# HiKapok/DAN

Measured on NVIDIA B200. Metric: images/sec anchor match+encode+decode+NMS @640^2, higher is better.
Workload: dtype f32

## Files before the change

### dan_b200/csrc/postprocess.cu

```cuda
#include <math.h>
#include <stdlib.h>
#include <string.h>

#include "common.cuh"

namespace dan {

#ifdef DAN_PHASE_TIMING
__device__ long long g_phase[32];
#define DAN_PHASE(slot) do { if (threadIdx.x == 0 && blockIdx.x == 0 && blockIdx.y == 0) g_phase[slot] = clock64(); } while (0)
#else
#define DAN_PHASE(slot) do { } while (0)
#endif

#ifndef DAN_PP_THREADS
#define DAN_PP_THREADS 1024
#endif
#define DAN_SORT_THREADS DAN_PP_THREADS
#include "sort.cuh"

struct PpArgs {
  const float* cls;
  const float4* loc;
  const float4* boxes;
  const float* ay0;
  const float* ax0;
  const float* ay1;
  const float* ax1;
  int n, batch, num_classes;
  float img_h, img_w;
  float select_thr, min_size_p1;
  float reject_below;
  float ps0, ps1, ps2, ps3;
  int keep_topk, nms_topk;
  int nms_cap;
  float nms_thr;
  int sort_bytes, kcap, wcap, cand_global, kept_global;
  int kstride;
  int dyn_smem_bytes;
  unsigned long long* keys;
  int32_t* key_count;
  int32_t* maybe;
  float4* stash;
  float* s_scores;
  float4* s_boxes;
  int32_t* s_index;
  unsigned long long* s_key;
  unsigned long long* s_key2;
  float4* s_box;
  float* s_area;
  float4* g_kept_box;
// ... 199 lines not shown
  r.area = fmul(fsub(r.y1, r.y0), fsub(r.x1, r.x0));
  return r;
}

__device__ __noinline__ bool nms_suppresses(float4 a, float a_area, float4 b, float b_area, float thr) {
  if (a_area <= 0.f || b_area <= 0.f) return false;
  const float h = fmaxf(fsub(fminf(a.z, b.z), fmaxf(a.x, b.x)), 0.f);
  const float w = fmaxf(fsub(fminf(a.w, b.w), fmaxf(a.y, b.y)), 0.f);
  const float inter = fmul(h, w);
  if (inter == 0.f) return 0.f > thr;
  return fdiv(inter, fsub(fadd(a_area, b_area), inter)) > thr;
}

DAN_D bool pair_suppresses(const float4& a, float a_area, const float4& b, float b_area, float thr) {
  if (thr >= 0.f) {
    const float h = fsub(fminf(a.z, b.z), fmaxf(a.x, b.x));
    const float w = fsub(fminf(a.w, b.w), fmaxf(a.y, b.y));
    if (!(h > 0.f && w > 0.f)) return false;
    if (!(a_area > 0.f && b_area > 0.f)) return false;
    const float inter = fmul(h, w);
    const float t = fmul(thr, fsub(fadd(a_area, b_area), inter));
    if (t > 1e-30f) {
      if (inter > fmul(t, 1.000001f)) return true;
      if (inter < fmul(t, 0.999999f)) return false;
    }
  }
  return nms_suppresses(a, a_area, b, b_area, thr);
}

DAN_D bool f2_maybe(const PpArgs& A, float x0, float x1) {
  return !(fsub(x1, x0) < A.reject_below) || fabsf(x0) > 1e5f || fabsf(x1) > 1e5f;
}

constexpr int kWin = kSortThreads;
#ifndef DAN_NMS_SURV
#define DAN_NMS_SURV 128
#endif
constexpr int kSurv = DAN_NMS_SURV;
constexpr int kSurvWords = kSurv / 32;
constexpr int kMaxSweeps = 12;
constexpr int kHintCells = 32 * 32;
constexpr size_t kGreedySmemMax = 186 * 1024;

struct GreedyPlan {
  size_t smem;
  int sort_bytes;
  int kcap;
  int wcap;
  int cand_global;
  int kept_global;
};

static int next_pow2(int64_t v) {
  int p = 1;
  while (p < v) p <<= 1;
  return p;
}

static GreedyPlan greedy_plan(int64_t n, int keep_topk, int nms_cap) {
  GreedyPlan g;
  const int sort_n = (int)(n < kSortCap ? (n > 0 ? n : 1) : kSortCap);
  g.sort_bytes = next_pow2(sort_n) * 8;
  g.kcap = (int)(keep_topk < n ? keep_topk : (n > 0 ? n : 1));
  g.wcap = (nms_cap + 31) / 32;
  const size_t kept_bytes = align_up((size_t)nms_cap * 16, 16) + 2 * align_up((size_t)nms_cap * 4, 16) + (size_t)64 * g.wcap * 4;
  const size_t cand_box = align_up((size_t)g.kcap * 16, 16);
  const size_t region0 = cand_box > (size_t)g.sort_bytes ? cand_box : (size_t)g.sort_bytes;
  const size_t full = region0 + align_up((size_t)g.kcap * 4, 16) + align_up((size_t)g.kcap * 8, 16) + kept_bytes;
  g.cand_global = g.kept_global = 0;
  g.smem = full;
  if (full > kGreedySmemMax) {
    g.cand_global = 1;
    g.smem = (size_t)g.sort_bytes + kept_bytes;
    if (g.smem > kGreedySmemMax) {
      g.kept_global = 1;
      g.smem = (size_t)g.sort_bytes;
    }
  }
  return g;
}

DAN_D void block_minmax(float lo, float hi, float& out_lo, float& out_hi) {
  __shared__ int s_lo[kSortThreads / 32], s_hi[kSortThreads / 32];
  const int lane = threadIdx.x & 31, warp = threadIdx.x >> 5;
  const int wl = __reduce_min_sync(0xffffffffu, float_to_ordered(lo));
  const int wh = __reduce_max_sync(0xffffffffu, float_to_ordered(hi));
  if (lane == 0) { s_lo[warp] = wl; s_hi[warp] = wh; }
  __syncthreads();
  int a = (lane < kSortThreads / 32) ? s_lo[lane] : 0x7fffffff, b = (lane < kSortThreads / 32) ? s_hi[lane] : (int)0x80000000;
  a = __reduce_min_sync(0xffffffffu, a);
  b = __reduce_max_sync(0xffffffffu, b);
  out_lo = ordered_to_float(a);
  out_hi = ordered_to_float(b);
  __syncthreads();
}

struct Stripes {
  float ylo, yinv, xlo, xinv;
  bool all;
  DAN_D static uint32_t axis(float v0, float v1, float lo, float inv) {
    const float f0 = (v0 - lo) * inv, f1 = (v1 - lo) * inv;
    if (!(fabsf(f0) < 1e9f) || !(fabsf(f1) < 1e9f)) return 0xffffffffu;
    const int s0 = min(max((int)f0, 0), 31), s1 = min(max((int)f1, 0), 31);
    return (0xffffffffu >> (31 - s1)) & (0xffffffffu << s0);
  }
  DAN_D uint2 masks(float4 bx, float area) const {
    if (!(area > 0.f)) return make_uint2(0u, 0u);
    if (all) return make_uint2(0xffffffffu, 0xffffffffu);
    return make_uint2(axis(bx.y, bx.w, xlo, xinv), axis(bx.x, bx.z, ylo, yinv));
  }
  DAN_D int cell(float4 bx) const {
    const float fy = ((bx.x + bx.z) * 0.5f - ylo) * yinv, fx = ((bx.y + bx.w) * 0.5f - xlo) * xinv;
    const int sy = (fabsf(fy) < 1e9f) ? min(max((int)fy, 0), 31) : 0;
    const int sx = (fabsf(fx) < 1e9f) ? min(max((int)fx, 0), 31) : 0;
    return sy * 32 + sx;
  }
};

DAN_D void bar_sync_chunk() { asm volatile("bar.sync 1, %0;" ::"n"(kSurv) : "memory"); }
DAN_D bool bar_or_chunk(bool pred) {
  int r;
  asm volatile(
      "{\n"
      "  .reg .pred p, q;\n"
      "  setp.ne.s32 q, %1, 0;\n"
      "  bar.red.or.pred p, 1, %2, q;\n"
      "  selp.s32 %0, 1, 0, p;\n"
      "}\n"
      : "=r"(r)
      : "r"((int)pred), "n"(kSurv)
      : "memory");
  return r != 0;
}

__device__ __noinline__ void resolve_chunk_serially(const uint32_t* T, uint32_t* keptm, uint32_t* supm, int ns) {
  const int lane = threadIdx.x & 31;
  uint32_t kw = (lane < kSurvWords) ? keptm[lane] : 0u;
  uint32_t sw = (lane < kSurvWords) ? supm[lane] : 0u;
  for (int v = 0; v < ns; ++v) {
    const int w = v >> 5;
    const uint32_t bit = 1u << (v & 31);
    const uint32_t known = __shfl_sync(0xffffffffu, kw | sw, w);
    if (known & bit) continue;
    const uint32_t t = (lane < kSurvWords && (lane << 5) < v) ? T[v * kSurvWords + lane] : 0u;
    const bool hit = __any_sync(0xffffffffu, (t & kw) != 0u);
    if (lane == w) {
      if (hit) sw |= bit;
      else kw |= bit;
    }
  }
  if (lane < kSurvWords) { keptm[lane] = kw; supm[lane] = sw; }
}

#ifndef DAN_NMS_REGS
#define DAN_NMS_BOUNDS __launch_bounds__(kSortThreads, 1024 / kSortThreads)
#else
#define DAN_NMS_BOUNDS __maxnreg__(DAN_NMS_REGS)
#endif
constexpr int kMaybeCap = 4096;

template <bool DECODE, int WHERE, bool FILTER>
__global__ void DAN_NMS_BOUNDS nms_greedy_kernel(const PpArgs A, const float* __restrict__ src_scores,
                                                                     const float4* __restrict__ src_boxes) {
  extern __shared__ __align__(16) unsigned char dyn_smem[];
  __shared__ SortScratch sc;
  __shared__ unsigned char s_alive[kWin];
  __shared__ unsigned short s_list[kWin];
  __shared__ int s_surv[kSurv];
  __shared__ float4 s_sbox[kSurv];
  __shared__ float s_sarea[kSurv];
  __shared__ uint32_t s_T[kSurv][kSurvWords];
  __shared__ uint32_t s_keptm[kSurvWords], s_supm[kSurvWords];
  __shared__ uint2 s_smask[kSurv];
  __shared__ int s_hint[2][kHintCells];
  __shared__ int s_wcnt[kSortThreads / 32];
  __shared__ int s_next[2];
  __shared__ int s_nlist, s_cnext;

  const int list = blockIdx.x;
  const int tid = threadIdx.x;
  const int lane = tid & 31;
  const int warp = tid >> 5;
  const unsigned lt_mask = (1u << lane) - 1u;
  const int b = list / max(A.num_classes - 1, 1);
  const int64_t o = (int64_t)list * A.kstride;
  const float thr = A.nms_thr;

  unsigned long long* keys = reinterpret_cast<unsigned long long*>(dyn_smem);
  float4* cbox;
  float* carea;
  uint2* cmask;
  unsigned char* p;
  if (WHERE >= 1) {
    cbox = A.s_box + o;
    carea = A.s_area + o;
    cmask = A.s_mask + o;
    p = dyn_smem + A.sort_bytes;
  } else {
    const size_t cand_box = ((size_t)A.kcap * 16 + 15) / 16 * 16;
    cbox = reinterpret_cast<float4*>(dyn_smem);
    carea = reinterpret_cast<float*>(dyn_smem + (cand_box > (size_t)A.sort_bytes ? cand_box : (size_t)A.sort_bytes));
    cmask = reinterpret_cast<uint2*>(reinterpret_cast<unsigned char*>(carea) + ((size_t)A.kcap * 4 + 15) / 16 * 16);
    p = reinterpret_cast<unsigned char*>(cmask) + ((size_t)A.kcap * 8 + 15) / 16 * 16;
  }
  float4* kbox;
  float* karea;
  int* krank;
  uint32_t* stripes;
// ... 2 lines not shown
    const int64_t ok = (int64_t)list * A.kstride;
    kbox = A.g_kept_box + ok;
    karea = A.g_kept_area + ok;
    krank = A.g_kept_rank + ok;
    stripes = A.g_stripes + (int64_t)list * 64 * ((A.kstride + 31) / 32);
  } else {
    kbox = reinterpret_cast<float4*>(p); p += ((size_t)A.nms_cap * 16 + 15) / 16 * 16;
    karea = reinterpret_cast<float*>(p); p += ((size_t)A.nms_cap * 4 + 15) / 16 * 16;
    krank = reinterpret_cast<int*>(p); p += ((size_t)A.nms_cap * 4 + 15) / 16 * 16;
    stripes = reinterpret_cast<uint32_t*>(p);
  }
  uint32_t* xs = stripes;
  uint32_t* ys = stripes + 32 * wcap;

  DAN_PHASE(0);
  unsigned long long* gkeys = A.keys + (int64_t)list * A.n;
  int cnt;
  if (FILTER) {
    __shared__ int s_maybe[kMaybeCap];
    __shared__ int s_nmaybe, s_nkeys;
    int* gmaybe = A.maybe + (int64_t)list * A.n;
    const int key_cap = A.sort_bytes / 8;
    if (tid == 0) { s_nmaybe = 0; s_nkeys = 0; }
    __syncthreads();
    auto put = [&](int pos, int a) {
      if (pos < kMaybeCap) s_maybe[pos] = a;
      else gmaybe[pos] = a;
    };
    auto push = [&](int a) { put(atomicAdd(&s_nmaybe, 1), a); };
    const float* x = A.cls + (int64_t)b * A.n * 2;
    const int head = (reinterpret_cast<uintptr_t>(x) & 15u) ? 1 : 0;
    const int nvec = (A.n - head) >> 1;
    const float4* xv = reinterpret_cast<const float4*>(x + 2 * head);
    for (int v0 = 0; v0 < nvec; v0 += 4 * kSortThreads) {
      float4 q[4];
#pragma unroll
      for (int u = 0; u < 4; ++u) {
        const int v = v0 + u * kSortThreads + tid;
        q[u] = (v < nvec) ? __ldcs(xv + v) : make_float4(0.f, 0.f, 0.f, 0.f);
      }
#pragma unroll
      for (int u = 0; u < 4; ++u) {
        const int v = v0 + u * kSortThreads + tid;
        const bool p0 = v < nvec && f2_maybe(A, q[u].x, q[u].y);
        const bool p1 = v < nvec && f2_maybe(A, q[u].z, q[u].w);
        const unsigned m0 = __ballot_sync(0xffffffffu, p0), m1 = __ballot_sync(0xffffffffu, p1);
        if ((m0 | m1) != 0u) {
          int base = 0;
          if (lane == 0) base = atomicAdd(&s_nmaybe, __popc(m0) + __popc(m1));
          base = __shfl_sync(0xffffffffu, base, 0);
          int pos = base + __popc(m0 & lt_mask) + __popc(m1 & lt_mask);
          if (p0) put(pos++, head + 2 * v);
          if (p1) put(pos, head + 2 * v + 1);
        }
      }
    }
    if (tid == 0 && head == 1 && f2_maybe(A, x[0], x[1])) push(0);
    if (tid == 1 && head + 2 * nvec < A.n && f2_maybe(A, x[2 * (A.n - 1)], x[2 * (A.n - 1) + 1])) push(A.n - 1);
    __syncthreads();
    const int nmaybe = s_nmaybe;
    for (int i0 = 0; i0 < nmaybe; i0 += kSortThreads) {
      const int i = i0 + tid;
      if (i < nmaybe) {
        const int a = (i < kMaybeCap) ? s_maybe[i] : gmaybe[i];
        const float2 xx = *reinterpret_cast<const float2*>(x + 2 * a);
        const float mx = fmaxf(xx.x, xx.y);
        const float e0 = cephes_expf(fsub(xx.x, mx));
        const float e1 = cephes_expf(fsub(xx.y, mx));
        const float pr = fmul(e1, fdiv(1.f, fadd(e0, e1)));
        if (pr > A.select_thr) {
          const float4 box = pp_box(A, b, a);
          if (A.stash != nullptr) A.stash[(int64_t)b * A.n + a] = box;
          const float w = fadd(fsub(box.w, box.y), 1.f);
          const float h = fadd(fsub(box.z, box.x), 1.f);
          if ((w > A.min_size_p1) && (h > A.min_size_p1)) {
            const unsigned long long key = ((unsigned long long)score_to_key(pr) << 32) | (unsigned long long)(0xFFFFFFFFu - (uint32_t)a);
            const int pos = atomicAdd(&s_nkeys, 1);
            if (pos < key_cap) keys[pos] = key;
            else gkeys[pos] = key;
          }
        }
      }
    }
    __syncthreads();
    cnt = s_nkeys;
    if (cnt > kSortCap) {
      for (int i = tid; i < min(cnt, key_cap); i += kSortThreads) gkeys[i] = keys[i];
      __syncthreads();
    }
  } else {
    cnt = min(A.key_count[list], A.n);
  }

  DAN_PHASE(8);
  const int k_want = min(A.keep_topk, cnt);
  int K;
  const unsigned long long* sorted = keys;
  if (k_want <= kSortCap) {
    unsigned long long* spare = ((size_t)A.sort_bytes + (size_t)min(cnt, kSortCap) * 8 <= (size_t)A.dyn_smem_bytes)
                                    ? reinterpret_cast<unsigned long long*>(dyn_smem + A.sort_bytes) : nullptr;
    K = min(select_and_sort(gkeys, cnt, k_want, keys, sc, FILTER, spare), A.keep_topk);
  } else {
    select_and_sort_large(gkeys, cnt, k_want, A.s_key + o, A.s_key2 + o, keys, sc);
    sorted = A.s_key + o;
    K = k_want;
  }
  DAN_PHASE(1);

  for (int r0 = K > 0 ? ((K - 1) / kSortThreads) * kSortThreads : -1; r0 >= 0; r0 -= kSortThreads) {
    const int r = r0 + tid;
    const unsigned long long key = (r < K) ? sorted[r] : 0ull;
    if (r < K) A.s_key[o + r] = key;
    __syncthreads();
    if (r < K) {
      const uint32_t idx = key_index(key);
      const NmsBox nb = nms_norm(DECODE ? (A.stash != nullptr ? A.stash[(int64_t)b * A.n + idx] : pp_box(A, b, (int)idx)) : src_boxes[idx]);
      cbox[r] = make_float4(nb.y0, nb.x0, nb.y1, nb.x1);
      carea[r] = nb.area;
    }
  }
  __syncthreads();
  DAN_PHASE(2);

#ifdef DAN_PHASE_TIMING
  long long acc[12] = {0, 0, 0, 0, 0, 0, 0, 0, 0, 0, 0, 0}, t_a = 0, t_b = 0, n_sweeps = 0, n_surv = 0, n_chunks = 0;
#define DAN_LAP(i) do { const long long now__ = clock64(); acc[i] += now__ - t_b; t_b = now__; } while (0)
#define DAN_TICK() (t_a = clock64())
#define DAN_TOCK(i) (acc[i] += clock64() - t_a)
#else
#define DAN_TICK() do { } while (0)
#define DAN_TOCK(i) do { } while (0)
#define DAN_LAP(i) do { } while (0)
#endif
  Stripes sg;
  {
    float ylo = 3.0e38f, yhi = -3.0e38f, xlo = 3.0e38f, xhi = -3.0e38f;
    for (int r = tid; r < K; r += kSortThreads) {
      const float4 bx = cbox[r];
      if (carea[r] > 0.f && fabsf(bx.x) < 1e30f && fabsf(bx.y) < 1e30f && fabsf(bx.z) < 1e30f && fabsf(bx.w) < 1e30f) {
        ylo = fminf(ylo, bx.x); yhi = fmaxf(yhi, bx.z);
        xlo = fminf(xlo, bx.y); xhi = fmaxf(xhi, bx.w);
      }
    }
    float ey, ex;
    block_minmax(ylo, yhi, sg.ylo, ey);
    block_minmax(xlo, xhi, sg.xlo, ex);
    sg.yinv = (ey > sg.ylo) ? 32.f / (ey - sg.ylo) : 0.f;
    sg.xinv = (ex > sg.xlo) ? 32.f / (ex - sg.xlo) : 0.f;
    sg.all = thr < 0.f;
  }
  for (int r = tid; r < K; r += kSortThreads) cmask[r] = sg.masks(cbox[r], carea[r]);
  for (int i = tid; i < 64 * wcap; i += kSortThreads) stripes[i] = 0u;
  for (int i = tid; i < 2 * kHintCells; i += kSortThreads) (&s_hint[0][0])[i] = 0x7fffffff;
  if (tid < 2) s_next[tid] = 0;
  if (tid == 0) s_nlist = 0;
  __syncthreads();
  int L = 0;
  int L_prev = 0;
  int w_end_prev = 0;
  for (int c0 = 0; c0 < K && L < A.nms_topk;) {
    const int w_end = min(K, c0 + kWin);
    DAN_TICK();
    const int my_r = c0 + tid;
    const bool in_win = my_r < w_end;
    {
      bool alive = false, search = false;
      int upto = 0;
      if (in_win) {
        const bool fresh = my_r >= w_end_prev;
        alive = fresh ? true : (s_alive[my_r & (kWin - 1)] != 0);
        upto = fresh ? 0 : L_prev;
      }
      if (alive && L > upto) {
        const uint2 mm = cmask[my_r];
        if (mm.x != 0u && mm.y != 0u) {
          const float4 me = cbox[my_r];
          const float my_area = carea[my_r];
          const int cl = sg.cell(me);
          const int h0 = s_hint[0][cl], h1 = s_hint[1][cl];
          bool dead = false;
          if (h0 >= upto && h0 < L) dead = pair_suppresses(kbox[h0], karea[h0], me, my_area, thr);
          if (!dead && h1 != h0 && h1 >= upto && h1 < L) dead = pair_suppresses(kbox[h1], karea[h1], me, my_area, thr);
          alive = !dead;
          search = !dead;
        }
      }
      if (in_win) s_alive[my_r & (kWin - 1)] = alive ? 1 : 0;
      const unsigned sm = __ballot_sync(0xffffffffu, search);
      int base = 0;
      if (lane == 0 && sm != 0u) base = atomicAdd(&s_nlist, __popc(sm));
      base = __shfl_sync(0xffffffffu, base, 0);
      if (search) s_list[base + __popc(sm & lt_mask)] = (unsigned short)tid;
    }
    __syncthreads();
    const int nlist = s_nlist;
    if (nlist > 0) {
      const int W = (L + 31) >> 5;
      const int G = W <= 8 ? 8 : (W <= 16 ? 16 : 32);
      const int cpw = 32 / G;
      const int gl = lane & (G - 1), sub = lane / G;
      const unsigned gmask = (G == 32 ? 0xffffffffu : ((1u << G) - 1u)) << (sub * G);
      while (true) {
        int i0 = 0;
        if (lane == 0) i0 = atomicAdd(&s_next[0], cpw);
        i0 = __shfl_sync(0xffffffffu, i0, 0);
        if (i0 >= nlist) break;
        const bool have = i0 + sub < nlist;
        const int r = c0 + (have ? (int)s_list[i0 + sub] : 0);
        const float4 me = have ? cbox[r] : make_float4(0.f, 0.f, 0.f, 0.f);
        const float my_area = have ? carea[r] : 0.f;
        const uint2 mm = have ? cmask[r] : make_uint2(0u, 0u);
        const int upto = (r >= w_end_prev) ? 0 : L_prev;
        bool sup = false;
        for (int wb = 0; wb < W; wb += G) {
          const int w = wb + gl;
          uint32_t poss = 0u;
          if (w < W && w >= (upto >> 5) && mm.x != 0u && mm.y != 0u) {
            uint32_t ax = 0u, ay = 0u;
            const int xe = 31 - __clz(mm.x), ye = 31 - __clz(mm.y);
#pragma unroll 2
            for (int st = __ffs(mm.x) - 1; st <= xe; ++st) ax |= xs[st * wcap + w];
#pragma unroll 2
            for (int st = __ffs(mm.y) - 1; st <= ye; ++st) ay |= ys[st * wcap + w];
            poss = ax & ay;
            if (w == (upto >> 5)) poss &= ~((1u << (upto & 31)) - 1u);
          }
          while (__any_sync(0xffffffffu, poss != 0u && !sup)) {
            bool t = false;
            if (poss != 0u && !sup) {
              const int j = (w << 5) + __ffs(poss) - 1;
              poss &= poss - 1u;
              t = pair_suppresses(kbox[j], karea[j], me, my_area, thr);
              if (t) atomicExch(&s_hint[1][sg.cell(me)], j);
            }
            if ((__ballot_sync(0xffffffffu, t) & gmask) != 0u) sup = true;
          }
        }
        if (have && gl == 0 && sup) s_alive[r & (kWin - 1)] = 0;
      }
    }
    __syncthreads();
    DAN_TOCK(0);
    DAN_TICK();
    const bool f = in_win && s_alive[my_r & (kWin - 1)] != 0;
    const unsigned fm = __ballot_sync(0xffffffffu, f);
    if (lane == 0) s_wcnt[warp] = __popc(fm);
    if (tid < kSurvWords) { s_keptm[tid] = 0u; s_supm[tid] = 0u; }
    __syncthreads();
    int total, ubase;
    {
      const int cw = (lane < kSortThreads / 32) ? s_wcnt[lane] : 0;
      int incl = cw;
#pragma unroll
      for (int d = 1; d < 32; d <<= 1) {
        const int up = __shfl_up_sync(0xffffffffu, incl, d);
        if (lane >= d) incl += up;
      }
      total = __shfl_sync(0xffffffffu, incl, 31);
      ubase = __shfl_sync(0xffffffffu, incl - cw, warp & 31);
    }
    if (f) {
      const int u = ubase + __popc(fm & lt_mask);
      if (u < kSurv) {
        s_surv[u] = my_r;
        s_sbox[u] = cbox[my_r];
        s_sarea[u] = carea[my_r];
        s_smask[u] = cmask[my_r];
        if (u == kSurv - 1) s_cnext = my_r + 1;
      }
    }
    __syncthreads();
    const int ns = min(total, kSurv);
    const int c_next = (total >= kSurv) ? s_cnext : w_end;
    DAN_TOCK(1);
    DAN_TICK();
    while (true) {
      int vi = 0;
      if (lane == 0) vi = atomicAdd(&s_next[1], 1);
      vi = __shfl_sync(0xffffffffu, vi, 0);
      if (vi >= ns) break;
      const int v = ns - 1 - vi;
      const float4 me = s_sbox[v];
      const float my_area = s_sarea[v];
      const uint2 mm = s_smask[v];
// ... 20 lines not shown
      const uint32_t vbit = 1u << (tid & 31);
      const bool mine = tid < ns;
#pragma unroll
      for (int w = 0; w < kSurvWords; ++w) T[w] = (mine && (w << 5) < tid) ? s_T[tid][w] : 0u;
      bool decided = !mine;
      bool open = true;
      while (open && sweeps < kMaxSweeps) {
        uint32_t hitm = 0u, pendm = 0u;
        if (!decided) {
#pragma unroll
          for (int w = 0; w < kSurvWords; ++w) {
            const uint32_t kw = s_keptm[w], sw = s_supm[w];
            hitm |= T[w] & kw;
            pendm |= T[w] & ~(kw | sw);
          }
        }
        bar_sync_chunk();
        if (!decided) {
          if (hitm != 0u) { atomicOr(&s_supm[vw], vbit); decided = true; }
          else if (pendm == 0u) { atomicOr(&s_keptm[vw], vbit); decided = true; }
        }
        open = bar_or_chunk(!decided);
        ++sweeps;
      }
      if (open) {
        if (warp == 0) resolve_chunk_serially(&s_T[0][0], s_keptm, s_supm, ns);
        bar_sync_chunk();
      }
      DAN_TOCK(3);
    }
    __syncthreads();
    DAN_TICK();
    {
      constexpr int kEntryThreads = kSortThreads / kSurv;
      const int v = tid / kEntryThreads, part = tid % kEntryThreads;
      const int vw = v >> 5;
      const uint32_t vbit = 1u << (v & 31);
      if (tid < 2) s_next[tid] = 0;
      if (tid == 2) s_nlist = 0;
      if (v < ns && (s_keptm[vw] & vbit)) {
        int before = 0;
#pragma unroll
        for (int w = 0; w < kSurvWords; ++w)
          if (w < vw) before += __popc(s_keptm[w]);
        const int pos = L + before + __popc(s_keptm[vw] & (vbit - 1u));
        if (pos < A.nms_topk) {
          const uint2 sm = s_smask[v];
          const uint32_t bit = 1u << (pos & 31);
          if (part == 0) {
            const float4 bx = s_sbox[v];
            kbox[pos] = bx;
            karea[pos] = s_sarea[v];
            krank[pos] = s_surv[v];
            if (sm.x != 0u) atomicMin(&s_hint[0][sg.cell(bx)], pos);
          }
          for (int st = part; st < 32; st += kEntryThreads) {
            if ((sm.x >> st) & 1u) atomicOr(&xs[st * wcap + (pos >> 5)], bit);
            if ((sm.y >> st) & 1u) atomicOr(&ys[st * wcap + (pos >> 5)], bit);
          }
        }
      }
    }
    __syncthreads();
    {
      int nk = 0;
#pragma unroll
      for (int w = 0; w < kSurvWords; ++w) nk += __popc(s_keptm[w]);
      L_prev = L;
      L = min(L + nk, A.nms_topk);
    }
    w_end_prev = w_end;
    c0 = c_next;
#ifdef DAN_PHASE_TIMING
    DAN_TOCK(4);
    n_sweeps += sweeps; n_surv += ns; ++n_chunks;
#endif
  }
  const int kept_n = L;
  DAN_PHASE(3);
#ifdef DAN_PHASE_TIMING
  if (threadIdx.x == 0 && blockIdx.x == 0) {
    for (int i = 0; i < 5; ++i) g_phase[10 + i] = acc[i];
    for (int i = 5; i < 12; ++i) g_phase[15 + i] = acc[i];
    g_phase[15] = n_sweeps; g_phase[16] = n_surv; g_phase[17] = n_chunks; g_phase[18] = K; g_phase[19] = kept_n;
  }
#endif

  auto put_score = [&](int64_t oo, float v) {
    A.out_scores[oo] = v;
    for (int q = 0; q < A.npeers; ++q) *reinterpret_cast<float*>(reinterpret_cast<char*>(A.out_scores + oo) + A.peer_delta[q]) = v;
  };
  auto put_box = [&](int64_t oo, float4 v) {
    A.out_boxes[oo] = v;
    for (int q = 0; q < A.npeers; ++q) *reinterpret_cast<float4*>(reinterpret_cast<char*>(A.out_boxes + oo) + A.peer_delta[q]) = v;
  };
  for (int t = tid; t < A.nms_topk; t += kSortThreads) {
    const int64_t oo = (int64_t)list * A.nms_topk + t;
    if (t < kept_n) {
      const int pos = krank[t];
      const unsigned long long key = A.s_key[o + pos];
      const uint32_t idx = key_index(key);
      put_score(oo, DECODE ? key_to_score((uint32_t)(key >> 32)) : src_scores[idx]);
      put_box(oo, DECODE ? kbox[t] : src_boxes[idx]);
      if (A.out_index != nullptr) A.out_index[oo] = (int32_t)idx;
      if (A.out_keep != nullptr) A.out_keep[oo] = A.filler ? pos : (int32_t)idx;
    } else {
      put_score(oo, 0.f);
      put_box(oo, make_float4(0.f, 0.f, 0.f, 0.f));
      if (A.out_index != nullptr) A.out_index[oo] = -1;
      if (A.out_keep != nullptr) {
        const int fpos = K + (t - kept_n);
        A.out_keep[oo] = (A.filler && fpos < A.keep_topk) ? fpos : -1;
      }
    }
  }
  if (tid == 0 && A.out_counts != nullptr) {
    A.out_counts[list] = kept_n;
    for (int q = 0; q < A.npeers; ++q) *reinterpret_cast<int32_t*>(reinterpret_cast<char*>(A.out_counts + list) + A.peer_delta[q]) = kept_n;
  }
  if (A.npeers > 0) {
    __threadfence_system();
    __syncthreads();
    if (tid == 0) {
      const int done = atomicAdd(A.peer_state, 1);
      if (done == (int)gridDim.x - 1) {
        A.peer_state[0] = 0;
        const int seq = A.peer_state[1] + 1;
        A.peer_state[1] = seq;
        __threadfence_system();
// ... 27 lines not shown
  w.key_count = take(lists * 4);
  w.keys = take(lists * n * 8);
  w.maybe = take(nms ? lists * n * 4 : 0);
  w.stash = take(stash_rows * 16);
  w.s_key = take(lists * ks * 8);
  w.s_key2 = take(lists * ks * 8);
  w.s_box = take(nms ? lists * ks * 16 : 0);
  w.s_area = take(nms ? lists * ks * 4 : 0);
  w.kept_box = take(nms ? lists * ks * 16 : 0);
  w.kept_area = take(nms ? lists * ks * 4 : 0);
  w.kept_rank = take(nms ? lists * ks * 4 : 0);
  w.s_mask = take(nms ? lists * ks * 8 : 0);
  w.stripes = take(nms ? lists * 64 * ((ks + 31) / 32) * 4 : 0);
  w.total = off;
  return w;
}

static void pp_bind(PpArgs& A, void* ws, const PpLayout& w) {
  char* base = static_cast<char*>(ws);
  A.key_count = reinterpret_cast<int32_t*>(base + w.key_count);
  A.keys = reinterpret_cast<unsigned long long*>(base + w.keys);
  A.maybe = reinterpret_cast<int32_t*>(base + w.maybe);
  A.s_key = reinterpret_cast<unsigned long long*>(base + w.s_key);
  A.s_key2 = reinterpret_cast<unsigned long long*>(base + w.s_key2);
  A.s_box = reinterpret_cast<float4*>(base + w.s_box);
  A.s_area = reinterpret_cast<float*>(base + w.s_area);
  A.g_kept_box = reinterpret_cast<float4*>(base + w.kept_box);
  A.g_kept_area = reinterpret_cast<float*>(base + w.kept_area);
  A.g_kept_rank = reinterpret_cast<int32_t*>(base + w.kept_rank);
  A.s_mask = reinterpret_cast<uint2*>(base + w.s_mask);
  A.g_stripes = reinterpret_cast<uint32_t*>(base + w.stripes);
}

template <bool DECODE, int WHERE, bool FILTER>
static int launch_greedy(const PpArgs& A, int lists, size_t smem, const float* src_scores, const float4* src_boxes, cudaStream_t st) {
  DAN_CUDA(cudaFuncSetAttribute(nms_greedy_kernel<DECODE, WHERE, FILTER>, cudaFuncAttributeMaxDynamicSharedMemorySize, (int)smem));
  nms_greedy_kernel<DECODE, WHERE, FILTER><<<lists, kSortThreads, smem, st>>>(A, src_scores, src_boxes);
  DAN_LAUNCH_CHECK("nms_greedy_kernel");
  return DAN_OK;
}

template <bool DECODE, bool FILTER>
static int run_sort_nms(const PpArgs& A_in, int lists, const float* src_scores, const float4* src_boxes, cudaStream_t st) {
  PpArgs A = A_in;
  const GreedyPlan g = greedy_plan(A.n, A.keep_topk, A.nms_cap);
  A.sort_bytes = g.sort_bytes;
  A.kcap = g.kcap;
  A.wcap = g.wcap;
  A.kstride = g.kcap;
  A.dyn_smem_bytes = (int)g.smem;
  A.cand_global = g.cand_global;
  A.kept_global = g.kept_global;
  if (g.kept_global) return launch_greedy<DECODE, 2, FILTER>(A, lists, g.smem, src_scores, src_boxes, st);
  if (g.cand_global) return launch_greedy<DECODE, 1, FILTER>(A, lists, g.smem, src_scores, src_boxes, st);
  return launch_greedy<DECODE, 0, FILTER>(A, lists, g.smem, src_scores, src_boxes, st);
}

}

using namespace dan;

extern "C" {

#ifdef DAN_PHASE_TIMING
int dan_debug_phases(long long* h_out32) { return cudaMemcpyFromSymbol(h_out32, g_phase, sizeof(long long) * 32) == cudaSuccess ? 0 : -3; }
#endif

size_t dan_postprocess_workspace_bytes(int32_t num_anchors, int32_t batch, int32_t num_classes, int32_t keep_topk) {
  if (num_anchors < 0 || batch < 0 || num_classes < 2 || keep_topk < 1) return 0;
  return pp_layout(num_anchors, (int64_t)batch * (num_classes - 1), keep_topk, true, (int64_t)batch * num_anchors).total;
}

size_t dan_sort_workspace_bytes(int64_t n, int32_t keep_topk) {
  if (n < 0 || keep_topk < 1) return 0;
  return pp_layout(n, 1, keep_topk, false).total;
}

size_t dan_nms_workspace_bytes(int64_t n, int32_t nms_topk) {
  if (n < 0 || nms_topk < 0) return 0;
  return pp_layout(n, 1, n > 0 ? n : 1, true).total;
}

static int postprocess_core(const dan_postprocess_params* p, const float* cls_pred, const float* loc_pred, const float* boxes_pred,
                            const float* a_ymin, const float* a_xmin, const float* a_ymax, const float* a_xmax, int32_t num_anchors,
                            int32_t batch, float* out_boxes, float* out_scores, int32_t* out_counts, int32_t* out_anchor_index,
// ... 229 lines not shown
```

### dan_b200/csrc/sort.cuh

```cuda
#pragma once

#ifndef DAN_PHASE
#define DAN_PHASE(slot) do { } while (0)
#endif

constexpr int kSortCap = 8192;
#ifndef DAN_SORT_THREADS
#define DAN_SORT_THREADS 1024
#endif
constexpr int kSortThreads = DAN_SORT_THREADS;

DAN_D uint32_t score_to_key(float s) { return (uint32_t)float_to_ordered(s) ^ 0x80000000u; }
DAN_D float key_to_score(uint32_t k) { return ordered_to_float((int)(k ^ 0x80000000u)); }

struct SortScratch {
  int hist[256];
  unsigned long long prefix;
  int remaining;
  int fill;
};

template <int KPT, int ST>
DAN_D void reg_stage(unsigned long long (&r)[KPT], int lsize, bool desc_t) {
  constexpr int LK = KPT == 32 ? 5 : KPT == 16 ? 4 : KPT == 8 ? 3 : KPT == 4 ? 2 : KPT == 2 ? 1 : 0;
#pragma unroll
  for (int e = 0; e < KPT; ++e) {
    if ((e & ST) == 0) {
      const bool desc = (lsize >= LK) ? desc_t : (((e >> lsize) & 1) == 0);
      const unsigned long long x = r[e], y = r[e | ST];
      if ((x < y) == desc) { r[e] = y; r[e | ST] = x; }
    }
  }
}

template <int KPT>
DAN_D void bitonic_sort_regs(unsigned long long* s_keys, int lp2) {
  constexpr int LK = KPT == 32 ? 5 : KPT == 16 ? 4 : KPT == 8 ? 3 : KPT == 4 ? 2 : KPT == 2 ? 1 : 0;
  const int tid = threadIdx.x;
  const int T = 1 << (lp2 - LK);
  const bool active = tid < T;
  unsigned long long r[KPT];
  if (active) {
#pragma unroll
// ... 14 lines not shown
          const bool keep_max = ((tid & (1 << (ls - LK))) == 0) == desc_t;
#pragma unroll
          for (int e = 0; e < KPT; ++e) {
            const unsigned long long o = s_keys[e * T + partner];
            r[e] = ((r[e] < o) == keep_max) ? o : r[e];
          }
        }
      } else if (!active) {
      } else if (ls >= LK) {
        const int lmask = 1 << (ls - LK);
        const bool keep_max = ((tid & lmask) == 0) == desc_t;
#pragma unroll
        for (int e = 0; e < KPT; ++e) {
          const unsigned long long o = __shfl_xor_sync(0xffffffffu, r[e], lmask);
          r[e] = ((r[e] < o) == keep_max) ? o : r[e];
        }
      } else {
        if constexpr (KPT > 16) { if (ls == 4) reg_stage<KPT, 16>(r, lsize, desc_t); }
        if constexpr (KPT > 8) { if (ls == 3) reg_stage<KPT, 8>(r, lsize, desc_t); }
        if constexpr (KPT > 4) { if (ls == 2) reg_stage<KPT, 4>(r, lsize, desc_t); }
        if constexpr (KPT > 2) { if (ls == 1) reg_stage<KPT, 2>(r, lsize, desc_t); }
        if constexpr (KPT > 1) { if (ls == 0) reg_stage<KPT, 1>(r, lsize, desc_t); }
      }
    }
  }
  __syncthreads();
  if (active) {
#pragma unroll
    for (int e = 0; e < KPT; ++e) s_keys[KPT * tid + e] = r[e];
  }
  __syncthreads();
}

DAN_D void sort_smem_keys(unsigned long long* s_keys, int m) {
  const int tid = threadIdx.x;
  int lp2 = 0;
  while ((1 << lp2) < m) ++lp2;
  const int p2 = 1 << lp2;
  for (int i = m + tid; i < p2; i += kSortThreads) s_keys[i] = 0ull;
  __syncthreads();
  if (lp2 >= 5) {
    constexpr int kLogThreads = kSortThreads == 1024 ? 10 : kSortThreads == 512 ? 9 : 8;
    const int lk = lp2 > kLogThreads ? lp2 - kLogThreads : 0;
    if (lk == 0) bitonic_sort_regs<1>(s_keys, lp2);
    else if (lk == 1) bitonic_sort_regs<2>(s_keys, lp2);
    else if (lk == 2) bitonic_sort_regs<4>(s_keys, lp2);
    else if (lk == 3) bitonic_sort_regs<8>(s_keys, lp2);
    else if (lk == 4) { if constexpr (kSortThreads < 1024) bitonic_sort_regs<16>(s_keys, lp2); }
    else { if constexpr (kSortThreads < 512) bitonic_sort_regs<32>(s_keys, lp2); }
    return;
  }
  for (int lsize = 1; lsize <= lp2; ++lsize) {
    for (int ls = lsize - 1; ls >= 0; --ls) {
      const int stride = 1 << ls;
      for (int t = tid; t < (p2 >> 1); t += kSortThreads) {
        const int lo = ((t >> ls) << (ls + 1)) | (t & (stride - 1));
        const int hi = lo | stride;
        const bool desc = ((lo >> lsize) & 1) == 0;
        const unsigned long long x = s_keys[lo], y = s_keys[hi];
        if ((x < y) == desc) { s_keys[lo] = y; s_keys[hi] = x; }
      }
      __syncthreads();
    }
  }
}

DAN_D void warp_sort_tile128(unsigned long long (&r)[4], int lane) {
  for (int lsize = 1; lsize <= 7; ++lsize) {
    const bool desc_t = ((lane >> (lsize >= 2 ? lsize - 2 : 0)) & 1) == 0;
    for (int ls = lsize - 1; ls >= 0; --ls) {
      if (ls >= 2) {
        const int lmask = 1 << (ls - 2);
        const bool keep_max = ((lane & lmask) == 0) == desc_t;
#pragma unroll
        for (int e = 0; e < 4; ++e) {
          const unsigned long long o = __shfl_xor_sync(0xffffffffu, r[e], lmask);
          r[e] = ((r[e] < o) == keep_max) ? o : r[e];
        }
      } else if (ls == 1) {
        reg_stage<4, 2>(r, lsize, desc_t);
      } else {
        reg_stage<4, 1>(r, lsize, desc_t);
      }
    }
  }
}

DAN_D void merge_sort_smem_keys(unsigned long long* s_a, unsigned long long* s_b, int m) {
  const int tid = threadIdx.x, lane = tid & 31, warp = tid >> 5;
  int rounds = 0;
  for (int run = 128; run < m; run <<= 1) ++rounds;
  unsigned long long* src = (rounds & 1) ? s_b : s_a;
  unsigned long long* dst = (rounds & 1) ? s_a : s_b;
  for (int t0 = warp * 128; t0 < m; t0 += (kSortThreads / 32) * 128) {
    unsigned long long r[4];
#pragma unroll
    for (int e = 0; e < 4; ++e) {
      const int i = t0 + 4 * lane + e;
      r[e] = (i < m) ? s_a[i] : 0ull;
    }
    warp_sort_tile128(r, lane);
    __syncwarp();
#pragma unroll
    for (int e = 0; e < 4; ++e) {
      const int i = t0 + 4 * lane + e;
      if (i < m) src[i] = r[e];
    }
  }
  __syncthreads();
  for (int run = 128; run < m; run <<= 1) {
    for (int i = tid; i < m; i += kSortThreads) {
      const int base = (i / (2 * run)) * (2 * run);
      const bool second = i - base >= run;
      const int x_lo = base + (second ? run : 0), y_lo = base + (second ? 0 : run);
      const int y_len = max(0, min(run, m - y_lo));
      const unsigned long long key = src[i];
      int lo = 0, hi = y_len;
      while (lo < hi) {
        const int mid = (lo + hi) >> 1;
        if (src[y_lo + mid] > key) lo = mid + 1;
        else hi = mid;
      }
      dst[base + (i - x_lo) + lo] = key;
    }
    __syncthreads();
    unsigned long long* t = src; src = dst; dst = t;
  }
}

DAN_D unsigned long long radix_select_kth(const unsigned long long* __restrict__ keys, int cnt, int k, SortScratch& sc) {
  const int tid = threadIdx.x;
  if (tid == 0) { sc.prefix = 0ull; sc.remaining = k; }
  unsigned long long prefix_mask = 0ull;
  for (int shift = 56; shift >= 0; shift -= 8) {
    for (int i = tid; i < 256; i += kSortThreads) sc.hist[i] = 0;
    __syncthreads();
    const unsigned long long prefix = sc.prefix;
    for (int i = tid; i < cnt; i += kSortThreads) {
      const unsigned long long key = keys[i];
      if ((key & prefix_mask) == prefix) atomicAdd(&sc.hist[(int)((key >> shift) & 255ull)], 1);
    }
    __syncthreads();
    if (tid == 0) {
      int cum = 0, bin = 255;
      for (; bin > 0; --bin) {
        if (cum + sc.hist[bin] >= sc.remaining) break;
        cum += sc.hist[bin];
      }
      sc.remaining -= cum;
      sc.prefix = prefix | ((unsigned long long)bin << shift);
    }
    prefix_mask |= 255ull << shift;
    __syncthreads();
  }
  return sc.prefix;
}

DAN_D int select_and_sort(const unsigned long long* __restrict__ keys, int cnt, int k, unsigned long long* s_keys, SortScratch& sc,
                          bool staged = false, unsigned long long* s_spare = nullptr) {
  const int tid = threadIdx.x;
  int m = cnt;
  if (cnt <= kSortCap) {
    if (!staged)
      for (int i = tid; i < cnt; i += kSortThreads) s_keys[i] = keys[i];
  } else {
    const unsigned long long kth = radix_select_kth(keys, cnt, k, sc);
    if (tid == 0) sc.fill = 0;
    __syncthreads();
    for (int i = tid; i < cnt; i += kSortThreads) {
      const unsigned long long key = keys[i];
      if (key >= kth) s_keys[atomicAdd(&sc.fill, 1)] = key;
    }
    m = k;
  }
  DAN_PHASE(8);
#ifdef DAN_NO_MERGE_SORT
  s_spare = nullptr;
#endif
  if (s_spare != nullptr && m > 128) {
    __syncthreads();
    merge_sort_smem_keys(s_keys, s_spare, m);
  } else {
    sort_smem_keys(s_keys, m);
  }
  return m;
}

DAN_D void select_and_sort_large(const unsigned long long* __restrict__ keys, int cnt, int k, unsigned long long* buf_a,
                                 unsigned long long* buf_b, unsigned long long* s_keys, SortScratch& sc) {
  const int tid = threadIdx.x;
  if (cnt > k) {
    const unsigned long long kth = radix_select_kth(keys, cnt, k, sc);
    if (tid == 0) sc.fill = 0;
    __syncthreads();
    for (int i = tid; i < cnt; i += kSortThreads) {
      const unsigned long long key = keys[i];
      if (key >= kth) buf_a[atomicAdd(&sc.fill, 1)] = key;
    }
  } else {
    for (int i = tid; i < k; i += kSortThreads) buf_a[i] = keys[i];
  }
  __syncthreads();
  for (int r0 = 0; r0 < k; r0 += kSortCap) {
    const int m = min(kSortCap, k - r0);
    for (int i = tid; i < m; i += kSortThreads) s_keys[i] = buf_a[r0 + i];
    __syncthreads();
    sort_smem_keys(s_keys, m);
    for (int i = tid; i < m; i += kSortThreads) buf_a[r0 + i] = s_keys[i];
    __syncthreads();
  }
  unsigned long long* src = buf_a;
  unsigned long long* dst = buf_b;
  for (long long run = kSortCap; run < k; run *= 2) {
    for (int i = tid; i < k; i += kSortThreads) {
      const long long base = (i / (2 * run)) * (2 * run);
      const bool second = i - base >= run;
      const long long x_lo = base + (second ? run : 0), y_lo = base + (second ? 0 : run);
      const long long y_len = max(0ll, min(run, (long long)k - y_lo));
      const unsigned long long key = src[i];
      long long lo = 0, hi = y_len;
      while (lo < hi) {
        const long long mid = (lo + hi) >> 1;
        if (src[y_lo + mid] > key) lo = mid + 1;
        else hi = mid;
      }
      dst[base + (i - x_lo) + lo] = key;
    }
    __syncthreads();
    unsigned long long* t = src; src = dst; dst = t;
  }
  if (src != buf_a) {
    for (int i = tid; i < k; i += kSortThreads) buf_a[i] = src[i];
    __syncthreads();
  }
}
```

Measured before the change: 702,600.

## Run greedy NMS with 512-thread CTAs, two per SM, smaller smem tiers

The greedy NMS kernel now uses 512-thread blocks with launch bounds for two CTAs per SM, instead of one 1024-thread CTA. To make room, the shared-memory budget drops to 86 KB, the sort cap to 4096 and the maybe-list cap to 2048, and the sort helpers are templated on thread count and cap. The intent is to overlap independent per-list work across two resident CTAs, which hides the many block-wide barriers in sort and NMS. In exchange, larger inputs may spill to the global-memory tiers or the radix-select path more often. Each CTA also has half the threads, and an optional debug occupancy check is added.

```diff
diff --git a/dan_b200/csrc/postprocess.cu b/dan_b200/csrc/postprocess.cu
--- a/dan_b200/csrc/postprocess.cu
+++ b/dan_b200/csrc/postprocess.cu
@@ -1,6 +1,9 @@
 #include <math.h>
+#include <stdio.h>
 #include <stdlib.h>
 #include <string.h>
+
+#include <atomic>
 
 #include "common.cuh"
 
@@ -13,10 +16,6 @@
 #define DAN_PHASE(slot) do { } while (0)
 #endif
 
-#ifndef DAN_PP_THREADS
-#define DAN_PP_THREADS 1024
-#endif
-#define DAN_SORT_THREADS DAN_PP_THREADS
 #include "sort.cuh"
 
 struct PpArgs {
@@ -282,7 +281,10 @@
   return !(fsub(x1, x0) < A.reject_below) || fabsf(x0) > 1e5f || fabsf(x1) > 1e5f;
 }
 
-constexpr int kWin = kSortThreads;
+constexpr int kGreedyThreads = 512;
+constexpr int kGreedyPerSm = 2;
+constexpr int kGreedySortCap = 4096;
+constexpr int kWin = kGreedyThreads;
 #ifndef DAN_NMS_SURV
 #define DAN_NMS_SURV 128
 #endif
@@ -290,7 +292,7 @@
 constexpr int kSurvWords = kSurv / 32;
 constexpr int kMaxSweeps = 12;
 constexpr int kHintCells = 32 * 32;
-constexpr size_t kGreedySmemMax = 186 * 1024;
+constexpr size_t kGreedySmemMax = 86 * 1024;
 
 struct GreedyPlan {
   size_t smem;
@@ -309,7 +311,7 @@
 
 static GreedyPlan greedy_plan(int64_t n, int keep_topk, int nms_cap) {
   GreedyPlan g;
-  const int sort_n = (int)(n < kSortCap ? (n > 0 ? n : 1) : kSortCap);
+  const int sort_n = (int)(n < kGreedySortCap ? (n > 0 ? n : 1) : kGreedySortCap);
   g.sort_bytes = next_pow2(sort_n) * 8;
   g.kcap = (int)(keep_topk < n ? keep_topk : (n > 0 ? n : 1));
   g.wcap = (nms_cap + 31) / 32;
@@ -330,14 +332,16 @@
   return g;
 }
 
+template <int NT>
 DAN_D void block_minmax(float lo, float hi, float& out_lo, float& out_hi) {
-  __shared__ int s_lo[kSortThreads / 32], s_hi[kSortThreads / 32];
+  static_assert(NT % 32 == 0 && NT <= 1024, "one partial per warp, reduced by one warp");
+  __shared__ int s_lo[NT / 32], s_hi[NT / 32];
   const int lane = threadIdx.x & 31, warp = threadIdx.x >> 5;
   const int wl = __reduce_min_sync(0xffffffffu, float_to_ordered(lo));
   const int wh = __reduce_max_sync(0xffffffffu, float_to_ordered(hi));
   if (lane == 0) { s_lo[warp] = wl; s_hi[warp] = wh; }
   __syncthreads();
-  int a = (lane < kSortThreads / 32) ? s_lo[lane] : 0x7fffffff, b = (lane < kSortThreads / 32) ? s_hi[lane] : (int)0x80000000;
+  int a = (lane < NT / 32) ? s_lo[lane] : 0x7fffffff, b = (lane < NT / 32) ? s_hi[lane] : (int)0x80000000;
   a = __reduce_min_sync(0xffffffffu, a);
   b = __reduce_max_sync(0xffffffffu, b);
   out_lo = ordered_to_float(a);
@@ -403,11 +407,11 @@
 }
 
 #ifndef DAN_NMS_REGS
-#define DAN_NMS_BOUNDS __launch_bounds__(kSortThreads, 1024 / kSortThreads)
+#define DAN_NMS_BOUNDS __launch_bounds__(kGreedyThreads, kGreedyPerSm)
 #else
 #define DAN_NMS_BOUNDS __maxnreg__(DAN_NMS_REGS)
 #endif
-constexpr int kMaybeCap = 4096;
+constexpr int kMaybeCap = 2048;
 
 template <bool DECODE, int WHERE, bool FILTER>
 __global__ void DAN_NMS_BOUNDS nms_greedy_kernel(const PpArgs A, const float* __restrict__ src_scores,
@@ -423,7 +427,7 @@
   __shared__ uint32_t s_keptm[kSurvWords], s_supm[kSurvWords];
   __shared__ uint2 s_smask[kSurv];
   __shared__ int s_hint[2][kHintCells];
-  __shared__ int s_wcnt[kSortThreads / 32];
+  __shared__ int s_wcnt[kGreedyThreads / 32];
   __shared__ int s_next[2];
   __shared__ int s_nlist, s_cnext;
 
@@ -492,16 +496,16 @@
     const int head = (reinterpret_cast<uintptr_t>(x) & 15u) ? 1 : 0;
     const int nvec = (A.n - head) >> 1;
     const float4* xv = reinterpret_cast<const float4*>(x + 2 * head);
-    for (int v0 = 0; v0 < nvec; v0 += 4 * kSortThreads) {
+    for (int v0 = 0; v0 < nvec; v0 += 4 * kGreedyThreads) {
       float4 q[4];
 #pragma unroll
       for (int u = 0; u < 4; ++u) {
-        const int v = v0 + u * kSortThreads + tid;
+        const int v = v0 + u * kGreedyThreads + tid;
         q[u] = (v < nvec) ? __ldcs(xv + v) : make_float4(0.f, 0.f, 0.f, 0.f);
       }
 #pragma unroll
       for (int u = 0; u < 4; ++u) {
-        const int v = v0 + u * kSortThreads + tid;
+        const int v = v0 + u * kGreedyThreads + tid;
         const bool p0 = v < nvec && f2_maybe(A, q[u].x, q[u].y);
         const bool p1 = v < nvec && f2_maybe(A, q[u].z, q[u].w);
         const unsigned m0 = __ballot_sync(0xffffffffu, p0), m1 = __ballot_sync(0xffffffffu, p1);
@@ -519,7 +523,7 @@
     if (tid == 1 && head + 2 * nvec < A.n && f2_maybe(A, x[2 * (A.n - 1)], x[2 * (A.n - 1) + 1])) push(A.n - 1);
     __syncthreads();
     const int nmaybe = s_nmaybe;
-    for (int i0 = 0; i0 < nmaybe; i0 += kSortThreads) {
+    for (int i0 = 0; i0 < nmaybe; i0 += kGreedyThreads) {
       const int i = i0 + tid;
       if (i < nmaybe) {
         const int a = (i < kMaybeCap) ? s_maybe[i] : gmaybe[i];
@@ -544,8 +548,8 @@
     }
     __syncthreads();
     cnt = s_nkeys;
-    if (cnt > kSortCap) {
-      for (int i = tid; i < min(cnt, key_cap); i += kSortThreads) gkeys[i] = keys[i];
+    if (cnt > kGreedySortCap) {
+      for (int i = tid; i < min(cnt, key_cap); i += kGreedyThreads) gkeys[i] = keys[i];
       __syncthreads();
     }
   } else {
@@ -556,18 +560,18 @@
   const int k_want = min(A.keep_topk, cnt);
   int K;
   const unsigned long long* sorted = keys;
-  if (k_want <= kSortCap) {
-    unsigned long long* spare = ((size_t)A.sort_bytes + (size_t)min(cnt, kSortCap) * 8 <= (size_t)A.dyn_smem_bytes)
+  if (k_want <= kGreedySortCap) {
+    unsigned long long* spare = ((size_t)A.sort_bytes + (size_t)min(cnt, kGreedySortCap) * 8 <= (size_t)A.dyn_smem_bytes)
                                     ? reinterpret_cast<unsigned long long*>(dyn_smem + A.sort_bytes) : nullptr;
-    K = min(select_and_sort(gkeys, cnt, k_want, keys, sc, FILTER, spare), A.keep_topk);
+    K = min(select_and_sort<kGreedyThreads, kGreedySortCap>(gkeys, cnt, k_want, keys, sc, FILTER, spare), A.keep_topk);
   } else {
-    select_and_sort_large(gkeys, cnt, k_want, A.s_key + o, A.s_key2 + o, keys, sc);
+    select_and_sort_large<kGreedyThreads, kGreedySortCap>(gkeys, cnt, k_want, A.s_key + o, A.s_key2 + o, keys, sc);
     sorted = A.s_key + o;
     K = k_want;
   }
   DAN_PHASE(1);
 
-  for (int r0 = K > 0 ? ((K - 1) / kSortThreads) * kSortThreads : -1; r0 >= 0; r0 -= kSortThreads) {
+  for (int r0 = K > 0 ? ((K - 1) / kGreedyThreads) * kGreedyThreads : -1; r0 >= 0; r0 -= kGreedyThreads) {
     const int r = r0 + tid;
     const unsigned long long key = (r < K) ? sorted[r] : 0ull;
     if (r < K) A.s_key[o + r] = key;
@@ -595,7 +599,7 @@
   Stripes sg;
   {
     float ylo = 3.0e38f, yhi = -3.0e38f, xlo = 3.0e38f, xhi = -3.0e38f;
-    for (int r = tid; r < K; r += kSortThreads) {
+    for (int r = tid; r < K; r += kGreedyThreads) {
       const float4 bx = cbox[r];
       if (carea[r] > 0.f && fabsf(bx.x) < 1e30f && fabsf(bx.y) < 1e30f && fabsf(bx.z) < 1e30f && fabsf(bx.w) < 1e30f) {
         ylo = fminf(ylo, bx.x); yhi = fmaxf(yhi, bx.z);
@@ -603,15 +607,15 @@
       }
     }
     float ey, ex;
-    block_minmax(ylo, yhi, sg.ylo, ey);
-    block_minmax(xlo, xhi, sg.xlo, ex);
+    block_minmax<kGreedyThreads>(ylo, yhi, sg.ylo, ey);
+    block_minmax<kGreedyThreads>(xlo, xhi, sg.xlo, ex);
     sg.yinv = (ey > sg.ylo) ? 32.f / (ey - sg.ylo) : 0.f;
     sg.xinv = (ex > sg.xlo) ? 32.f / (ex - sg.xlo) : 0.f;
     sg.all = thr < 0.f;
   }
-  for (int r = tid; r < K; r += kSortThreads) cmask[r] = sg.masks(cbox[r], carea[r]);
-  for (int i = tid; i < 64 * wcap; i += kSortThreads) stripes[i] = 0u;
-  for (int i = tid; i < 2 * kHintCells; i += kSortThreads) (&s_hint[0][0])[i] = 0x7fffffff;
+  for (int r = tid; r < K; r += kGreedyThreads) cmask[r] = sg.masks(cbox[r], carea[r]);
+  for (int i = tid; i < 64 * wcap; i += kGreedyThreads) stripes[i] = 0u;
+  for (int i = tid; i < 2 * kHintCells; i += kGreedyThreads) (&s_hint[0][0])[i] = 0x7fffffff;
   if (tid < 2) s_next[tid] = 0;
   if (tid == 0) s_nlist = 0;
   __syncthreads();
@@ -656,7 +660,7 @@
     const int nlist = s_nlist;
     if (nlist > 0) {
       const int W = (L + 31) >> 5;
-      const int G = W <= 8 ? 8 : (W <= 16 ? 16 : 32);
+      const int G = W <= 4 ? 4 : (W <= 8 ? 8 : (W <= 16 ? 16 : 32));
       const int cpw = 32 / G;
       const int gl = lane & (G - 1), sub = lane / G;
       const unsigned gmask = (G == 32 ? 0xffffffffu : ((1u << G) - 1u)) << (sub * G);
@@ -709,7 +713,7 @@
     __syncthreads();
     int total, ubase;
     {
-      const int cw = (lane < kSortThreads / 32) ? s_wcnt[lane] : 0;
+      const int cw = (lane < kGreedyThreads / 32) ? s_wcnt[lane] : 0;
       int incl = cw;
 #pragma unroll
       for (int d = 1; d < 32; d <<= 1) {
@@ -796,7 +800,7 @@
     __syncthreads();
     DAN_TICK();
     {
-      constexpr int kEntryThreads = kSortThreads / kSurv;
+      constexpr int kEntryThreads = kGreedyThreads / kSurv;
       const int v = tid / kEntryThreads, part = tid % kEntryThreads;
       const int vw = v >> 5;
       const uint32_t vbit = 1u << (v & 31);
@@ -858,7 +862,7 @@
     A.out_boxes[oo] = v;
     for (int q = 0; q < A.npeers; ++q) *reinterpret_cast<float4*>(reinterpret_cast<char*>(A.out_boxes + oo) + A.peer_delta[q]) = v;
   };
-  for (int t = tid; t < A.nms_topk; t += kSortThreads) {
+  for (int t = tid; t < A.nms_topk; t += kGreedyThreads) {
     const int64_t oo = (int64_t)list * A.nms_topk + t;
     if (t < kept_n) {
       const int pos = krank[t];
@@ -952,10 +956,29 @@
   A.g_stripes = reinterpret_cast<uint32_t*>(base + w.stripes);
 }
 
+static bool debug_checks() {
+  const char* e = getenv("DAN_B200_DEBUG");
+  return e != nullptr && e[0] != '\0';
+}
+
 template <bool DECODE, int WHERE, bool FILTER>
 static int launch_greedy(const PpArgs& A, int lists, size_t smem, const float* src_scores, const float4* src_boxes, cudaStream_t st) {
-  DAN_CUDA(cudaFuncSetAttribute(nms_greedy_kernel<DECODE, WHERE, FILTER>, cudaFuncAttributeMaxDynamicSharedMemorySize, (int)smem));
-  nms_greedy_kernel<DECODE, WHERE, FILTER><<<lists, kSortThreads, smem, st>>>(A, src_scores, src_boxes);
+  auto* kern = nms_greedy_kernel<DECODE, WHERE, FILTER>;
+  DAN_CUDA(cudaFuncSetAttribute(kern, cudaFuncAttributeMaxDynamicSharedMemorySize, (int)kGreedySmemMax));
+  if (debug_checks()) {
+    static std::atomic<unsigned long long> checked{0ull};
+    int dev = 0;
+    DAN_CUDA(cudaGetDevice(&dev));
+    const unsigned long long bit = 1ull << (dev & 63);
+    if ((checked.load() & bit) == 0ull) {
+      int per_sm = 0;
+      DAN_CUDA(cudaOccupancyMaxActiveBlocksPerMultiprocessor(&per_sm, kern, kGreedyThreads, kGreedySmemMax));
+      DAN_REQUIRE(per_sm >= kGreedyPerSm, DAN_ERR_UNSUPPORTED, "nms_greedy_kernel<%d, %d, %d>: %d CTAs per SM at %zu bytes of dynamic shared memory, planned %d",
+                  (int)DECODE, WHERE, (int)FILTER, per_sm, kGreedySmemMax, kGreedyPerSm);
+      checked.fetch_or(bit);
+    }
+  }
+  kern<<<lists, kGreedyThreads, smem, st>>>(A, src_scores, src_boxes);
   DAN_LAUNCH_CHECK("nms_greedy_kernel");
   return DAN_OK;
 }
@@ -971,6 +994,9 @@
   A.dyn_smem_bytes = (int)g.smem;
   A.cand_global = g.cand_global;
   A.kept_global = g.kept_global;
+  if (debug_checks())
+    fprintf(stderr, "dan_b200 nms_greedy plan: n %d keep_topk %d nms_cap %d -> tier %d sort_bytes %d smem %zu\n", A.n, A.keep_topk,
+            A.nms_cap, g.kept_global ? 2 : g.cand_global ? 1 : 0, g.sort_bytes, g.smem);
   if (g.kept_global) return launch_greedy<DECODE, 2, FILTER>(A, lists, g.smem, src_scores, src_boxes, st);
   if (g.cand_global) return launch_greedy<DECODE, 1, FILTER>(A, lists, g.smem, src_scores, src_boxes, st);
   return launch_greedy<DECODE, 0, FILTER>(A, lists, g.smem, src_scores, src_boxes, st);
diff --git a/dan_b200/csrc/sort.cuh b/dan_b200/csrc/sort.cuh
--- a/dan_b200/csrc/sort.cuh
+++ b/dan_b200/csrc/sort.cuh
@@ -5,10 +5,7 @@
 #endif
 
 constexpr int kSortCap = 8192;
-#ifndef DAN_SORT_THREADS
-#define DAN_SORT_THREADS 1024
-#endif
-constexpr int kSortThreads = DAN_SORT_THREADS;
+constexpr int kSortThreads = 1024;
 
 DAN_D uint32_t score_to_key(float s) { return (uint32_t)float_to_ordered(s) ^ 0x80000000u; }
 DAN_D float key_to_score(uint32_t k) { return ordered_to_float((int)(k ^ 0x80000000u)); }
@@ -89,28 +86,30 @@
   __syncthreads();
 }
 
+template <int NT = kSortThreads, int CAP = kSortCap>
 DAN_D void sort_smem_keys(unsigned long long* s_keys, int m) {
   const int tid = threadIdx.x;
   int lp2 = 0;
   while ((1 << lp2) < m) ++lp2;
   const int p2 = 1 << lp2;
-  for (int i = m + tid; i < p2; i += kSortThreads) s_keys[i] = 0ull;
+  for (int i = m + tid; i < p2; i += NT) s_keys[i] = 0ull;
   __syncthreads();
   if (lp2 >= 5) {
-    constexpr int kLogThreads = kSortThreads == 1024 ? 10 : kSortThreads == 512 ? 9 : 8;
+    constexpr int kLogThreads = NT == 1024 ? 10 : NT == 512 ? 9 : 8;
+    constexpr int kMaxKpt = CAP / NT;
     const int lk = lp2 > kLogThreads ? lp2 - kLogThreads : 0;
     if (lk == 0) bitonic_sort_regs<1>(s_keys, lp2);
-    else if (lk == 1) bitonic_sort_regs<2>(s_keys, lp2);
-    else if (lk == 2) bitonic_sort_regs<4>(s_keys, lp2);
-    else if (lk == 3) bitonic_sort_regs<8>(s_keys, lp2);
-    else if (lk == 4) { if constexpr (kSortThreads < 1024) bitonic_sort_regs<16>(s_keys, lp2); }
-    else { if constexpr (kSortThreads < 512) bitonic_sort_regs<32>(s_keys, lp2); }
+    else if (lk == 1) { if constexpr (kMaxKpt >= 2) bitonic_sort_regs<2>(s_keys, lp2); }
+    else if (lk == 2) { if constexpr (kMaxKpt >= 4) bitonic_sort_regs<4>(s_keys, lp2); }
+    else if (lk == 3) { if constexpr (kMaxKpt >= 8) bitonic_sort_regs<8>(s_keys, lp2); }
+    else if (lk == 4) { if constexpr (kMaxKpt >= 16) bitonic_sort_regs<16>(s_keys, lp2); }
+    else { if constexpr (kMaxKpt >= 32) bitonic_sort_regs<32>(s_keys, lp2); }
     return;
   }
   for (int lsize = 1; lsize <= lp2; ++lsize) {
     for (int ls = lsize - 1; ls >= 0; --ls) {
       const int stride = 1 << ls;
-      for (int t = tid; t < (p2 >> 1); t += kSortThreads) {
+      for (int t = tid; t < (p2 >> 1); t += NT) {
         const int lo = ((t >> ls) << (ls + 1)) | (t & (stride - 1));
         const int hi = lo | stride;
         const bool desc = ((lo >> lsize) & 1) == 0;
@@ -143,13 +142,14 @@
   }
 }
 
+template <int NT = kSortThreads>
 DAN_D void merge_sort_smem_keys(unsigned long long* s_a, unsigned long long* s_b, int m) {
   const int tid = threadIdx.x, lane = tid & 31, warp = tid >> 5;
   int rounds = 0;
   for (int run = 128; run < m; run <<= 1) ++rounds;
   unsigned long long* src = (rounds & 1) ? s_b : s_a;
   unsigned long long* dst = (rounds & 1) ? s_a : s_b;
-  for (int t0 = warp * 128; t0 < m; t0 += (kSortThreads / 32) * 128) {
+  for (int t0 = warp * 128; t0 < m; t0 += (NT / 32) * 128) {
     unsigned long long r[4];
 #pragma unroll
     for (int e = 0; e < 4; ++e) {
@@ -166,7 +166,7 @@
   }
   __syncthreads();
   for (int run = 128; run < m; run <<= 1) {
-    for (int i = tid; i < m; i += kSortThreads) {
+    for (int i = tid; i < m; i += NT) {
       const int base = (i / (2 * run)) * (2 * run);
       const bool second = i - base >= run;
       const int x_lo = base + (second ? run : 0), y_lo = base + (second ? 0 : run);
@@ -185,15 +185,16 @@
   }
 }
 
+template <int NT = kSortThreads>
 DAN_D unsigned long long radix_select_kth(const unsigned long long* __restrict__ keys, int cnt, int k, SortScratch& sc) {
   const int tid = threadIdx.x;
   if (tid == 0) { sc.prefix = 0ull; sc.remaining = k; }
   unsigned long long prefix_mask = 0ull;
   for (int shift = 56; shift >= 0; shift -= 8) {
-    for (int i = tid; i < 256; i += kSortThreads) sc.hist[i] = 0;
+    for (int i = tid; i < 256; i += NT) sc.hist[i] = 0;
     __syncthreads();
     const unsigned long long prefix = sc.prefix;
-    for (int i = tid; i < cnt; i += kSortThreads) {
+    for (int i = tid; i < cnt; i += NT) {
       const unsigned long long key = keys[i];
       if ((key & prefix_mask) == prefix) atomicAdd(&sc.hist[(int)((key >> shift) & 255ull)], 1);
     }
@@ -213,18 +214,19 @@
   return sc.prefix;
 }
 
+template <int NT = kSortThreads, int CAP = kSortCap>
 DAN_D int select_and_sort(const unsigned long long* __restrict__ keys, int cnt, int k, unsigned long long* s_keys, SortScratch& sc,
                           bool staged = false, unsigned long long* s_spare = nullptr) {
   const int tid = threadIdx.x;
   int m = cnt;
-  if (cnt <= kSortCap) {
+  if (cnt <= CAP) {
     if (!staged)
-      for (int i = tid; i < cnt; i += kSortThreads) s_keys[i] = keys[i];
+      for (int i = tid; i < cnt; i += NT) s_keys[i] = keys[i];
   } else {
-    const unsigned long long kth = radix_select_kth(keys, cnt, k, sc);
+    const unsigned long long kth = radix_select_kth<NT>(keys, cnt, k, sc);
     if (tid == 0) sc.fill = 0;
     __syncthreads();
-    for (int i = tid; i < cnt; i += kSortThreads) {
+    for (int i = tid; i < cnt; i += NT) {
       const unsigned long long key = keys[i];
       if (key >= kth) s_keys[atomicAdd(&sc.fill, 1)] = key;
     }
@@ -236,40 +238,41 @@
 #endif
   if (s_spare != nullptr && m > 128) {
     __syncthreads();
-    merge_sort_smem_keys(s_keys, s_spare, m);
+    merge_sort_smem_keys<NT>(s_keys, s_spare, m);
   } else {
-    sort_smem_keys(s_keys, m);
+    sort_smem_keys<NT, CAP>(s_keys, m);
   }
   return m;
 }
 
+template <int NT = kSortThreads, int CAP = kSortCap>
 DAN_D void select_and_sort_large(const unsigned long long* __restrict__ keys, int cnt, int k, unsigned long long* buf_a,
                                  unsigned long long* buf_b, unsigned long long* s_keys, SortScratch& sc) {
   const int tid = threadIdx.x;
   if (cnt > k) {
-    const unsigned long long kth = radix_select_kth(keys, cnt, k, sc);
+    const unsigned long long kth = radix_select_kth<NT>(keys, cnt, k, sc);
     if (tid == 0) sc.fill = 0;
     __syncthreads();
-    for (int i = tid; i < cnt; i += kSortThreads) {
+    for (int i = tid; i < cnt; i += NT) {
       const unsigned long long key = keys[i];
       if (key >= kth) buf_a[atomicAdd(&sc.fill, 1)] = key;
     }
   } else {
-    for (int i = tid; i < k; i += kSortThreads) buf_a[i] = keys[i];
-  }
-  __syncthreads();
-  for (int r0 = 0; r0 < k; r0 += kSortCap) {
-    const int m = min(kSortCap, k - r0);
-    for (int i = tid; i < m; i += kSortThreads) s_keys[i] = buf_a[r0 + i];
-    __syncthreads();
-    sort_smem_keys(s_keys, m);
-    for (int i = tid; i < m; i += kSortThreads) buf_a[r0 + i] = s_keys[i];
+    for (int i = tid; i < k; i += NT) buf_a[i] = keys[i];
+  }
+  __syncthreads();
+  for (int r0 = 0; r0 < k; r0 += CAP) {
+    const int m = min(CAP, k - r0);
+    for (int i = tid; i < m; i += NT) s_keys[i] = buf_a[r0 + i];
+    __syncthreads();
+    sort_smem_keys<NT, CAP>(s_keys, m);
+    for (int i = tid; i < m; i += NT) buf_a[r0 + i] = s_keys[i];
     __syncthreads();
   }
   unsigned long long* src = buf_a;
   unsigned long long* dst = buf_b;
-  for (long long run = kSortCap; run < k; run *= 2) {
-    for (int i = tid; i < k; i += kSortThreads) {
+  for (long long run = CAP; run < k; run *= 2) {
+    for (int i = tid; i < k; i += NT) {
       const long long base = (i / (2 * run)) * (2 * run);
       const bool second = i - base >= run;
       const long long x_lo = base + (second ? run : 0), y_lo = base + (second ? 0 : run);
@@ -287,7 +290,7 @@
     unsigned long long* t = src; src = dst; dst = t;
   }
   if (src != buf_a) {
-    for (int i = tid; i < k; i += kSortThreads) buf_a[i] = src[i];
-    __syncthreads();
-  }
-}
+    for (int i = tid; i < k; i += NT) buf_a[i] = src[i];
+    __syncthreads();
+  }
+}
```

After: 718,500, median of 6. 2.3% higher.
